# Signalsmith-Audio/signalsmith-stretch

Measured on AMD Instinct MI355X. Metric: Msamples/sec (in+out) at 48kHz stereo presetDefault, higher is better.
Workload: dtype f32

## Files before the change

### signalsmith-stretch_amd/csrc/smst_fft.hip

```cpp
#include "smst_kernels_common.h"
#include <type_traits>

namespace smst {

template <int SIGN> __device__ __forceinline__ fc mulTwiddle(fc v, fc w) { return fmul<(SIGN > 0)>(v, w); }
template <int SIGN> __device__ __forceinline__ fc addJ(fc a, fc b) { return (SIGN < 0) ? fsubI(a, b) : faddI(a, b); }
template <int SIGN> __device__ __forceinline__ fc subJ(fc a, fc b) { return (SIGN < 0) ? faddI(a, b) : fsubI(a, b); }
template <int SIGN> __device__ __forceinline__ fc mulJ(fc a) { return (SIGN < 0) ? fmake(a.y, -a.x) : fmake(-a.y, a.x); }

template <int SIGN>
__device__ __forceinline__ void dft4(fc &a, fc &b, fc &c, fc &d) {
	const fc apc = fadd(a, c), amc = fsub(a, c), bpd = fadd(b, d), bmd = fsub(b, d);
	a = fadd(apc, bpd);
	b = addJ<SIGN>(amc, bmd);
	c = fsub(apc, bpd);
	d = subJ<SIGN>(amc, bmd);
}
template <int SIGN>
__device__ __forceinline__ void dft4J(fc &a, fc &b, fc &c, fc &d) {
	const fc apc = addJ<SIGN>(a, c), amc = subJ<SIGN>(a, c), bpd = fadd(b, d), bmd = fsub(b, d);
	a = fadd(apc, bpd);
	b = addJ<SIGN>(amc, bmd);
	c = fsub(apc, bpd);
	d = subJ<SIGN>(amc, bmd);
}
template <int SIGN>
__device__ __forceinline__ void dft3(fc &a, fc &b, fc &c) {
	const float s3 = 0.86602540378443864676f;
	const fc bpc = fadd(b, c), bmc = fsub(b, c);
	const fc t = fmake(a.x - 0.5f*bpc.x, a.y - 0.5f*bpc.y);
	const fc jb = mulJ<SIGN>(bmc);
	const fc u = fmake(jb.x*s3, jb.y*s3);
	a = fadd(a, bpc);
	b = fadd(t, u);
	c = fsub(t, u);
}
template <int SIGN>
__device__ __forceinline__ void dft5(fc &a, fc &b, fc &c, fc &d, fc &e) {
	const float c1 = 0.30901699437494742410f, c2 = -0.80901699437494742410f;
	const float s1 = 0.95105651629515357212f, s2 = 0.58778525229247312917f;
	const fc bpe = fadd(b, e), bme = fsub(b, e), cpd = fadd(c, d), cmd = fsub(c, d);
	const fc t1 = fmake(a.x + c1*bpe.x + c2*cpd.x, a.y + c1*bpe.y + c2*cpd.y);
	const fc t2 = fmake(a.x + c2*bpe.x + c1*cpd.x, a.y + c2*bpe.y + c1*cpd.y);
	const fc u1 = fmake(s1*bme.x + s2*cmd.x, s1*bme.y + s2*cmd.y);
	const fc u2 = fmake(s2*bme.x - s1*cmd.x, s2*bme.y - s1*cmd.y);
	a = fadd(a, fadd(bpe, cpd));
	b = addJ<SIGN>(t1, u1);
	c = addJ<SIGN>(t2, u2);
	d = subJ<SIGN>(t2, u2);
	e = subJ<SIGN>(t1, u1);
}
template <int SIGN>
__device__ float2 *fftLds(float2 *src2, float2 *dst2, const FftPlan &plan, const float2 *__restrict__ tw2) {
	fc *src = reinterpret_cast<fc *>(src2), *dst = reinterpret_cast<fc *>(dst2);
	const fc *__restrict__ tw = reinterpret_cast<const fc *>(tw2);
	const int H = plan.H;
	int nCur = H;
	int shift = 0;
	for (int pass = 0; pass < plan.npass; ++pass) {
		const int r = plan.radix[pass];
		const int m = nCur/r;
		const int nb = H/r;
		const int twScale = H/nCur;
		if (r == 4) {
			const int s = 1 << shift;
			for (int t = threadIdx.x; t < nb; t += blockDim.x) {
				const int p = t >> shift, q0 = t & (s - 1);
				const fc *in = src + q0 + (p << shift);
				const int inStride = m << shift;
				fc *out = dst + q0 + ((4*p) << shift);
				fc a = in[0], b = in[inStride], c = in[2*inStride], e = in[3*inStride];
				dft4<SIGN>(a, b, c, e);
				const int ti = p*twScale;
				out[0] = a;
				out[s] = mulTwiddle<SIGN>(b, tw[ti]);
				out[2*s] = mulTwiddle<SIGN>(c, tw[2*ti]);
				out[3*s] = mulTwiddle<SIGN>(e, tw[3*ti]);
			}
			shift += 2;
		} else if (r == 2) {
			const int s = 1 << shift;
			for (int t = threadIdx.x; t < nb; t += blockDim.x) {
				const int p = t >> shift, q0 = t & (s - 1);
				const fc *in = src + q0 + (p << shift);
				const int inStride = m << shift;
				fc *out = dst + q0 + ((2*p) << shift);
				const fc a = in[0], b = in[inStride];
				out[0] = fadd(a, b);
				out[s] = mulTwiddle<SIGN>(fsub(a, b), tw[p*twScale]);
			}
			shift += 1;
		} else if (r == 3) {
			const int s = nb;
			for (int t = threadIdx.x; t < nb; t += blockDim.x) {
				fc a = src[t], b = src[t + s], c = src[t + 2*s];
				dft3<SIGN>(a, b, c);
				dst[t] = a;
				dst[t + s] = b;
				dst[t + 2*s] = c;
			}
		} else {
			const int s = nb;
			for (int t = threadIdx.x; t < nb; t += blockDim.x) {
				fc a = src[t], b = src[t + s], c = src[t + 2*s], e = src[t + 3*s], f = src[t + 4*s];
				dft5<SIGN>(a, b, c, e, f);
				dst[t] = a;
				dst[t + s] = b;
				dst[t + 2*s] = c;
				dst[t + 3*s] = e;
				dst[t + 4*s] = f;
			}
		}
		__syncthreads();
		fc *tmp = src; src = dst; dst = tmp;
		nCur = m;
	}
	return reinterpret_cast<float2 *>(src);
}

template <int SIGN>
__device__ __forceinline__ fc mulConst(fc v, float re, float im) {
	const float s = (SIGN < 0) ? -im : im;
	return fmake(v.x*re - v.y*s, v.x*s + v.y*re);
}
template <int SIGN>
__device__ __forceinline__ void dft16(fc (&v)[16]) {
#pragma unroll
	for (int i = 0; i < 4; ++i) dft4<SIGN>(v[i], v[i + 4], v[i + 8], v[i + 12]);
	const float c1 = 0.92387953251128675613f, s1 = 0.38268343236508977173f, h = 0.70710678118654752440f;
	v[1 + 4] = mulConst<SIGN>(v[1 + 4], c1, s1);
	v[1 + 8] = mulConst<SIGN>(v[1 + 8], h, h);
	v[1 + 12] = mulConst<SIGN>(v[1 + 12], s1, c1);
	v[2 + 4] = mulConst<SIGN>(v[2 + 4], h, h);
	v[2 + 12] = mulConst<SIGN>(v[2 + 12], -h, h);
	v[3 + 4] = mulConst<SIGN>(v[3 + 4], s1, c1);
	v[3 + 8] = mulConst<SIGN>(v[3 + 8], -h, h);
	v[3 + 12] = mulConst<SIGN>(v[3 + 12], -c1, -s1);
#pragma unroll
	for (int e = 0; e < 4; ++e) {
		if (e == 2) dft4J<SIGN>(v[4*e], v[4*e + 1], v[4*e + 2], v[4*e + 3]);
		else dft4<SIGN>(v[4*e], v[4*e + 1], v[4*e + 2], v[4*e + 3]);
	}
}
template <int SIGN, int RA, int N>
__device__ __forceinline__ void dftPow2(fc (&v)[N], int base, int stride) {
	if constexpr (RA == 2) {
		const fc a = v[base], b = v[base + stride];
		v[base] = fadd(a, b);
		v[base + stride] = fsub(a, b);
	} else if constexpr (RA == 4) {
		dft4<SIGN>(v[base], v[base + stride], v[base + 2*stride], v[base + 3*stride]);
	} else {
		static_assert(RA == 8, "radix 2, 4 or 8");
		fc e0 = v[base], e1 = v[base + 2*stride], e2 = v[base + 4*stride], e3 = v[base + 6*stride];
		fc o0 = v[base + stride], o1 = v[base + 3*stride], o2 = v[base + 5*stride], o3 = v[base + 7*stride];
		dft4<SIGN>(e0, e1, e2, e3);
		dft4<SIGN>(o0, o1, o2, o3);
		const float h = 0.70710678118654752440f;
		o1 = mulConst<SIGN>(o1, h, h);
		o3 = mulConst<SIGN>(o3, -h, h);
		v[base] = fadd(e0, o0); v[base + 4*stride] = fsub(e0, o0);
		v[base + stride] = fadd(e1, o1); v[base + 5*stride] = fsub(e1, o1);
		v[base + 2*stride] = addJ<SIGN>(e2, o2); v[base + 6*stride] = subJ<SIGN>(e2, o2);
		v[base + 3*stride] = fadd(e3, o3); v[base + 7*stride] = fsub(e3, o3);
	}
}
template <int R3> struct LastStage {
	static constexpr int G = (R3%3 == 0) ? 3 : 5;
	static constexpr int RA = R3/G;
	static_assert(R3%G == 0 && (RA == 2 || RA == 4 || RA == 8), "last stage: {2,4,8} x {3,5} points");
};
template <int SIGN, int R3>
__device__ __forceinline__ void dftLast(fc (&v)[R3]) {
	constexpr int G = LastStage<R3>::G, RA = LastStage<R3>::RA;
#pragma unroll
	for (int i = 0; i < G; ++i) dftPow2<SIGN, RA>(v, i, G);
#pragma unroll
	for (int i = 1; i < G; ++i) {
#pragma unroll
		for (int e = 1; e < RA; ++e) {
			const float ang = 6.28318530717958647692f*float(i*e)/float(R3);
			v[i + G*e] = mulConst<SIGN>(v[i + G*e], __builtin_cosf(ang), __builtin_sinf(ang));
		}
	}
#pragma unroll
	for (int e = 0; e < RA; ++e) {
		if constexpr (G == 3) dft3<SIGN>(v[G*e], v[G*e + 1], v[G*e + 2]);
		else dft5<SIGN>(v[G*e], v[G*e + 1], v[G*e + 2], v[G*e + 3 < R3 ? G*e + 3 : 0], v[G*e + 4 < R3 ? G*e + 4 : 0]);
	}
}

struct BlockSync { __device__ __forceinline__ void operator()() const { __syncthreads(); } };
struct NoHook { __device__ __forceinline__ void operator()() const {} };
struct NoArrival { __device__ __forceinline__ fc operator()(fc v, int) const { return v; } };
template <int FRAMES> struct FrameSet { fc f[FRAMES]; };
struct StageTwiddles { float4 w[8]; };
struct TwiddlesFromTable {};
template <int SIGN, int R3, bool LEAN, int ROUNDS = 0, int FRAMES = 1, typename Load, typename Prep, typename Store, typename Sync = BlockSync, typename LastRead = NoHook,
          typename Requested = NoHook, typename FirstWritten = NoHook, typename Arrived = NoArrival, typename TwRegs = TwiddlesFromTable>
__device__ __forceinline__ void fftFast(float2 *lds2, const float4 *__restrict__ twA, const float4 *__restrict__ twB, Load load, Prep prep, Store store,
                                        const int t = threadIdx.x, Sync sync = Sync(), LastRead lastRead = LastRead(), Requested requested = Requested(),
                                        FirstWritten firstWritten = FirstWritten(), Arrived arrived = Arrived(), TwRegs twRegs = TwRegs()) {
	static_assert(FRAMES == 1 || FRAMES == 2, "one frame, or two in lockstep");
	constexpr int MA = 16*R3, BUF = 17*MA;
	constexpr bool TW_REGS = std::is_same<TwRegs, StageTwiddles>::value;
	static_assert(!(TW_REGS && LEAN), "the lean tables have no register form");
	fc *lds = reinterpret_cast<fc *>(lds2);
	auto prepOf = [&](int j, int idx, int f) { if constexpr (FRAMES == 1) return prep(j, idx); else return prep(j, idx, f); };
	auto storeOf = [&](int j, fc u, auto r, int idx, int f) { if constexpr (FRAMES == 1) store(j, u, r, idx); else store(j, u, r, idx, f); };
	fc v[FRAMES][16];
	if (t < MA) {
#pragma unroll
		for (int k = 0; k < 16; ++k) {
			if constexpr (FRAMES == 1) v[0][k] = load(t + MA*k, k);
			else {
				const FrameSet<FRAMES> both = load(t + MA*k, k);
#pragma unroll
				for (int f = 0; f < FRAMES; ++f) v[f][k] = both.f[f];
			}
		}
	}
	requested();
	if (t < MA) {
#pragma unroll
		for (int f = 0; f < FRAMES; ++f) {
#pragma unroll
			for (int k = 0; k < 16; ++k) {
				if constexpr (FRAMES == 1) v[f][k] = arrived(v[f][k], t + MA*k);
				else v[f][k] = arrived(v[f][k], t + MA*k, k, f);
			}
		}
		fc w[16];
		if constexpr (LEAN) {
			const float4 a = twA[t], b = twA[MA + t], c = twA[2*MA + t];
			w[1] = fmake(a.x, a.y); w[2] = fmake(a.z, a.w); w[3] = fmake(b.x, b.y); w[4] = fmake(b.z, b.w);
			w[8] = fmake(c.x, c.y); w[12] = fmake(c.z, c.w);
#pragma unroll
			for (int hi = 4; hi <= 12; hi += 4) {
#pragma unroll
				for (int lo = 1; lo < 4; ++lo) w[hi + lo] = fmul<false>(w[hi], w[lo]);
			}
		} else {
			float4 wA[8];
#pragma unroll
			for (int i = 0; i < 8; ++i) {
				if constexpr (TW_REGS) wA[i] = twRegs.w[i];
				else wA[i] = twA[i*MA + t];
			}
#pragma unroll
			for (int n = 1; n < 16; ++n) {
				const float4 pr = wA[(n - 1) >> 1];
				w[n] = ((n - 1) & 1) ? fmake(pr.z, pr.w) : fmake(pr.x, pr.y);
			}
		}
#pragma unroll
		for (int f = 0; f < FRAMES; ++f) dft16<SIGN>(v[f]);
#pragma unroll
		for (int f = 0; f < FRAMES; ++f) {
#pragma unroll
			for (int pos = 0; pos < 16; ++pos) {
				const int n = (pos >> 2) + 4*(pos & 3);
				lds[f*BUF + 17*t + n] = n > 0 ? mulTwiddle<SIGN>(v[f][pos], w[n]) : v[f][pos];
			}
		}
	}
	firstWritten();
	sync();
	const int p = t >> 4, q0 = t & 15;
	if (t < MA) {
#pragma unroll
		for (int f = 0; f < FRAMES; ++f) {
#pragma unroll
			for (int k = 0; k < 16; ++k) v[f][k] = lds[f*BUF + q0 + 17*(p + R3*k)];
		}
	}
	sync();
	if (t < MA) {
		float4 wB[8];
#pragma unroll
		for (int i = 0; i < 8; ++i) wB[i] = twB[i*R3 + p];
#pragma unroll
		for (int f = 0; f < FRAMES; ++f) dft16<SIGN>(v[f]);
#pragma unroll
		for (int f = 0; f < FRAMES; ++f) {
#pragma unroll
			for (int pos = 0; pos < 16; ++pos) {
				const int n = (pos >> 2) + 4*(pos & 3);
				fc val = v[f][pos];
				if (n > 0) {
					const float4 pr = wB[(n - 1) >> 1];
					val = mulTwiddle<SIGN>(val, ((n - 1) & 1) ? fmake(pr.z, pr.w) : fmake(pr.x, pr.y));
				}
				lds[f*BUF + q0 + 256*p + 16*n] = val;
			}
		}
	}
	sync();
	if (t < 256) {
		constexpr int G = LastStage<R3>::G, RA = LastStage<R3>::RA;
		fc u[FRAMES][R3];
#pragma unroll
		for (int f = 0; f < FRAMES; ++f) {
#pragma unroll
			for (int k = 0; k < R3; ++k) u[f][k] = lds[f*BUF + t + 256*k];
		}
		lastRead();
		constexpr int CHUNK = ROUNDS ? R3/ROUNDS : (R3 <= 12 ? R3 : (R3 == 24 ? 6 : 5));
		decltype(prepOf(0, 0, 0)) ready[FRAMES][CHUNK];
#pragma unroll
		for (int f = 0; f < FRAMES; ++f) {
#pragma unroll
			for (int i = 0; i < CHUNK; ++i) {
				const int e = i/G, c = i - G*e;
				ready[f][i] = prepOf(t + 256*(e + RA*c), e + RA*c, f);
			}
		}
#pragma unroll
		for (int f = 0; f < FRAMES; ++f) dftLast<SIGN, R3>(u[f]);
#pragma unroll
		for (int f = 0; f < FRAMES; ++f) {
#pragma unroll
			for (int p0 = 0; p0 < R3; p0 += CHUNK) {
				if (p0 > 0) {
#pragma unroll
					for (int i = 0; i < CHUNK; ++i) {
						const int pos = p0 + i, e = pos/G, c = pos - G*e;
						if (pos < R3) ready[f][i] = prepOf(t + 256*(e + RA*c), e + RA*c, f);
					}
				}
#pragma unroll
				for (int i = 0; i < CHUNK; ++i) {
					const int pos = p0 + i, e = pos/G, c = pos - G*e;
					if (pos < R3) storeOf(t + 256*(e + RA*c), u[f][pos], ready[f][i], e + RA*c, f);
				}
			}
		}
	}
}

constexpr int fastBlockThreads(int R3) { return 16*R3 > 256 ? 16*R3 : 256; }

__device__ __forceinline__ bool hopWantsAnalysis(const HopDesc &hd, int which) {
	return (hd.flags & HOP_ACTIVE) && (hd.flags & HOP_NEW_SPECTRUM) && !(hd.flags & HOP_PREANALYSED) && (!which || (hd.flags & HOP_REANALYSE_PREV));
}

__device__ __forceinline__ int halfBinIndex(int j, int H, int N) {
	const int kk = 2*j;
	return kk >= H ? N - 1 - kk : kk;
}
__device__ __forceinline__ fc loadHalfBin(const float2 *X, int j, int H, int N) {
	return fconjLoad(X + halfBinIndex(j, H, N), 2*j >= H);
}
__device__ __forceinline__ void storeHalfBin(float2 *dst, int j, fc u, int H, int N) {
	fconjStore(dst + halfBinIndex(j, H, N), u, 2*j >= H);
}

__device__ __forceinline__ float2 analysisElement(float4 w, float xr, float xi, int slot) {
	float2 r = make_float2(0.f, 0.f);
	if (slot < 15) r = make_float2(xr*w.x, xr*w.y);
	if (slot > 0) r = make_float2(fmaf(xi, w.z, r.x), fmaf(xi, w.w, r.y));
	return r;
}
__device__ __forceinline__ float2 analysisSamples(const float *x0, const float *x1, int m, int slot) {
	return make_float2(slot < 15 ? x0[m] : 0.f, slot > 0 ? x1[m] : 0.f);
}
__device__ __forceinline__ float2 analysisElement(float4 w, const float *x0, const float *x1, int m, int slot) {
	const float2 x = analysisSamples(x0, x1, m, slot);
	return analysisElement(w, x.x, x.y, slot);
}
__device__ __forceinline__ fc leanModulation(float2 hb, int k, int per) {
	const float ang = 3.14159265358979323846f*float(k)/float(per);
	return fmulExpr(fpack(hb), fmake(__builtin_cosf(ang), -__builtin_sinf(ang)));
}
__device__ __forceinline__ void storeWindowed(float *dst, int m, fc u, fc tw, float wRe, float wIm, int B, int H) {
	const int halfB = B/2;
	const fc v = fmulc(u, tw);
	if (m < B - halfB) dst[m + halfB] = (2*v.x)*wRe;
	if (m >= H - halfB) dst[m - H + halfB] = (2*v.y)*wIm;
}
__device__ __forceinline__ void storeWindowed(float *dst, int m, fc u, float4 r, int B, int H) {
	storeWindowed(dst, m, u, fmake(r.x, r.y), r.z, r.w, B, H);
}

template <int R3, bool LEAN>
__global__ __launch_bounds__(fastBlockThreads(R3)) __attribute__((amdgpu_waves_per_eu(4, 4))) void kAnalyseFast(DevBatch d, IoArgs io, int sBase, int hopBase, int lateOnly) {
	extern __shared__ __attribute__((aligned(16))) unsigned char smemRaw[];
	float2 *lds = reinterpret_cast<float2 *>(smemRaw);
	const BlockCoord bc = xcdAwareBlock();
	const int k = bc.x;
	const int c = bc.y >> 1;
	const int which = bc.y & 1;
	const int s = bc.s;
	const HopDesc hd = d.hops[(size_t)(sBase + s)*d.hopStride + hopBase + k];
	if (!hopWantsAnalysis(hd, which)) return;
	if (lateOnly && analysisWindowInCall(d.B, d.M, d.I, hd.inputOffset, which, io.inSamples[sBase + s])) return;
	const int B = d.B, H = d.M, halfB = B/2, N = d.N;
	const int base = hd.inputOffset - (which ? d.I : 0) - B;
	const float *x = io.in + (size_t)(sBase + s)*io.inStreamStride + (size_t)c*io.inChannelStride;
	const float *hist = d.hist + ((size_t)(sBase + s)*d.C + c)*(size_t)d.histPitch + d.histBase[d.histCur][sBase + s] + d.histLen;
	const float2 *__restrict__ winA = d.winA, *__restrict__ winB = d.winB;
	float2 *dst = (which ? d.Xprev : d.Xcur) + rowOf(d, s, k, c);
	auto prep = [](int, int) { return 0; };
	auto store = [&](int j, fc u, int, int) { storeHalfBin(dst, j, u, H, N); };
	constexpr int MA = 16*R3;
	const float4 *__restrict__ twA = LEAN ? d.twA6 : d.twA4;
	const float2 *__restrict__ win2 = d.win2;
	const float2 hb = LEAN ? d.halfTw[min((int)threadIdx.x, MA - 1)] : make_float2(0.f, 0.f);
	if (base >= 0 && H - halfB == MA && B - halfB == 15*MA) {
		const float *x0 = x + base + halfB, *x1 = x + base - H + halfB;
		const float4 *__restrict__ win4 = d.win4;
		fftFast<-1, R3, LEAN>(lds, twA, d.twB4,
			[&](int m, int slot) {
				if constexpr (LEAN) {
					const float2 w = win2[m];
					float2 z = make_float2(0.f, 0.f);
					if (slot < 15) z.x = x0[m]*w.x;
					if (slot > 0) z.y = x1[m]*w.y;
					return fmul<false>(fpack(z), leanModulation(hb, slot, 32));
				} else {
					return fpack(analysisElement(win4[m], x0, x1, m, slot));
				}
// ... 150 lines not shown
		}
		if (!on[0] && !on[1]) continue;
		auto prep = [](int, int, int = 0) { return 0; };
		if (on[0] && on[1]) {
			float4 win[16];
			[[maybe_unused]] fc landed[TWIST ? R3 : 1];
			fftFast<-1, R3, false, 0, 2>(wg.lds, nullptr, wg.twB,
				[&](int m, int slot) {
					FrameSet<2> r;
#pragma unroll
					for (int f = 0; f < 2; ++f) r.f[f] = fpack(analysisSamples(x0[f], x1[f], m, slot));
					return r;
				},
				prep, [&](int j, fc u, int, int idx, int f) {
					if constexpr (TWIST) {
						const fc landedValue = fconjIf(u, 2*j >= H);
						float2 *row = dst[f] + halfBinIndex(j, H, N);
						if (f == 0) { landed[idx] = landedValue; *reinterpret_cast<fc *>(row) = landedValue; }
						else *row = prevHopTwist(funpack(landed[idx]), funpack(landedValue), rotOf[idx]);
					} else {
						storeHalfBin(dst[f], j, u, H, N);
					}
				}, t, sync, NoHook(),
				[&]() {
#pragma unroll
					for (int slot = 0; slot < 16; ++slot) win[slot] = wg.table[tA + MA*slot];
					asm volatile("" ::: "memory");
				},
				NoHook(), [&](fc x, int, int slot, int) { return fpack(analysisElement(win[slot], x.x, x.y, slot)); }, twA);
		} else {
			const int f = on[0] ? 0 : 1;
			const float *xa = x0[f], *xb = x1[f];
			float2 *dstOne = dst[f];
			fftFast<-1, R3, false>(wg.lds, nullptr, wg.twB,
				[&](int m, int slot) { return fpack(analysisElement(wg.table[tA + MA*slot], xa, xb, m, slot)); },
				prep, [&](int j, fc u, int, int) { storeHalfBin(dstOne, j, u, H, N); }, t, sync, NoHook(), NoHook(), NoHook(), NoArrival(), twA);
		}
		sync();
	}
}

__global__ __launch_bounds__(256) void kTwistRows(DevBatch d, IoArgs io, int sBase, int hopBase, int teams) {
	const int k = blockIdx.x, c = blockIdx.y, s = blockIdx.z;
	const HopDesc hd = d.hops[(size_t)(sBase + s)*d.hopStride + hopBase + k];
	if (!hopWantsAnalysis(hd, 1)) return;
	const int nIn = io.inSamples[sBase + s];
	if (teams && analysisWindowInCall(d.B, d.M, d.I, hd.inputOffset, 0, nIn) && analysisWindowInCall(d.B, d.M, d.I, hd.inputOffset, 1, nIn)) return;
	const float2 *cur = d.Xcur + rowOf(d, s, k, c);
	float2 *prev = d.Xprev + rowOf(d, s, k, c);
	for (int b = threadIdx.x; b < d.M; b += blockDim.x) prev[b] = prevHopTwist(cur[b], prev[b], d.rot[b]);
}

template <int R3, bool LEAN>
__global__ __launch_bounds__(fastBlockThreads(R3)) void kSynthFast(DevBatch d, int sBase, int hopBase) {
	extern __shared__ __attribute__((aligned(16))) unsigned char smemRaw[];
	float2 *lds = reinterpret_cast<float2 *>(smemRaw);
	const int k = blockIdx.x, c = blockIdx.y, s = blockIdx.z;
	const HopDesc hd = d.hops[(size_t)(sBase + s)*d.hopStride + hopBase + k];
	if (!(hd.flags & HOP_ACTIVE)) return;
	const int B = d.B, H = d.M, N = d.N;
	const float2 *X = d.OUT + rowOf(d, s, k, c);
	float *__restrict__ frame = frameOf(d, s, k, c);
	auto loadBin = [&](int j, int) { return loadHalfBin(X, j, H, N); };
	if constexpr (LEAN) {
		const float2 *__restrict__ win2 = d.win2;
		const float2 hb = d.halfTw[min((int)threadIdx.x, 255)];
		fftFast<+1, R3, true>(lds, d.twA6, d.twB4, loadBin,
			[&](int m, int) { return win2[m]; },
			[&](int m, fc u, float2 w, int j) { storeWindowed(frame, m, u, leanModulation(hb, j, 2*R3), w.x, w.y, B, H); });
	} else {
		const float4 *__restrict__ synTab = d.synTab;
		fftFast<+1, R3, false>(lds, d.twA4, d.twB4, loadBin,
			[&](int m, int) {
				return synTab[m];
			},
			[&](int m, fc u, float4 r, int) { storeWindowed(frame, m, u, r, B, H); });
	}
}

template <int R3, int TEAMS>
__global__ __launch_bounds__(256*TEAMS) void kSynthTeams(DevBatch d, const HopDesc *__restrict__ hopTable, int sBase, int hopBase, int tileHops, int nStreams) {
	extern __shared__ __attribute__((aligned(16))) unsigned char smemRaw[];
	constexpr int H = 256*R3, N = 2*H;
	const int B = d.B;
	const int total = tileHops*d.C*nStreams;
	TeamWorkgroup<R3, TEAMS> wg(smemRaw, d, d.synTab);
	const TeamSync sync = wg.sync();
	const int stride = gridDim.x*TEAMS;
	for (int lin = blockIdx.x + gridDim.x*wg.team; lin < total; lin += stride) {
		const BlockCoord bc = xcdAwareCoord(lin, tileHops, d.C, nStreams);
		const HopDesc hd = hopTable[(size_t)(sBase + bc.s)*d.hopStride + hopBase + bc.x];
		if (!(hd.flags & HOP_ACTIVE)) continue;
		const float2 *X = d.OUT + rowOf(d, bc.s, bc.x, bc.y);
		float *__restrict__ frame = frameOf(d, bc.s, bc.x, bc.y);
		fftFast<+1, R3, false>(wg.lds, wg.twA, wg.twB,
			[&](int j, int) { return loadHalfBin(X, j, H, N); },
			[&](int m, int) { return wg.table[m]; },
			[&](int m, fc u, float4 r, int) { storeWindowed(frame, m, u, r, B, H); }, wg.t, sync);
		sync();
	}
}

__device__ __forceinline__ float carriedSumAt(const DevBatch &d, size_t row, int i) { return i < d.carryLen ? loadCarrySum(d, d.carryCur, row + i) : 0.0f; }
__device__ __forceinline__ float carriedProductAt(const DevBatch &d, const float *__restrict__ carryWpOld, int i) { return i < d.carryLen ? carryWpOld[i] : 1e-30f; }
struct FrameRange { int lo, hi; };
__device__ __forceinline__ FrameRange coveringFrames(int relFirst, int relLast, int B, int I, int hopCount) {
	FrameRange r;
	r.hi = (relLast >= 0) ? relLast/I : -1;
	r.lo = (relFirst - B + 1 > 0) ? (relFirst - B + 1 + I - 1)/I : 0;
	if (r.hi > hopCount - 1) r.hi = hopCount - 1;
	return r;
}
__device__ __forceinline__ float windowProductAt(const DevBatch &d, const EmitDesc &ed, const float *__restrict__ carryWpOld, int i) {
	float wp = carriedProductAt(d, carryWpOld, i);
	if (ed.hopCount > 0) {
		const int rel = ed.nLo + i - ed.firstHopPos - d.delta;
		const FrameRange q = coveringFrames(rel, rel, d.B, d.I, ed.hopCount);
		for (int k = q.lo; k <= q.hi; ++k) wp += d.wprod[rel - k*d.I];
	}
	return wp;
}
__global__ __launch_bounds__(256) void kEmitProducts(DevBatch d, int sBase, int tileIndex) {
	const int sg = sBase + blockIdx.y;
	const EmitDesc ed = d.emit[(size_t)sg*d.emitStride + tileIndex];
	const int span = ed.nHi - ed.nLo, CL = d.carryLen;
	const float *carryWpOld = d.carryWp[d.carryCur] + carryWpRow(d, sg) + d.carryBase[d.carryCur][sg];
	const int i = blockIdx.x*blockDim.x + threadIdx.x;
	if (i == 0) d.carryBase[d.carryCur ^ 1][sg] = 0;
	if (i < d.wpHeadLen) d.wpHead[(size_t)sg*d.wpHeadLen + i] = windowProductAt(d, ed, carryWpOld, i);
	else if (i - d.wpHeadLen < CL) d.carryWp[d.carryCur ^ 1][carryWpRow(d, sg) + (i - d.wpHeadLen)] = windowProductAt(d, ed, carryWpOld, span + (i - d.wpHeadLen));
}

struct SynthEmitEdge {
	EmitDesc ed;
	float *out;
	size_t carryRow;
	size_t carried;
	const float *wpOld;
};
__device__ __forceinline__ SynthEmitEdge synthEmitEdge(const DevBatch &d, const IoArgs &io, int sg, int c, int tileIndex) {
	SynthEmitEdge e;
	e.ed = d.emit[(size_t)sg*d.emitStride + tileIndex];
	const int carryFrom = d.carryBase[d.carryCur][sg];
	e.carryRow = carrySumRow(d, sg, c);
	e.carried = e.carryRow + carryFrom;
	e.wpOld = d.carryWp[d.carryCur] + carryWpRow(d, sg) + carryFrom;
	e.out = io.out + (size_t)sg*io.outStreamStride + (size_t)c*io.outChannelStride;
	return e;
}
__device__ __forceinline__ void synthEmitPlace(const DevBatch &d, const SynthEmitEdge &e, int n, float sum, float wp) {
	if (n < e.ed.nHi) e.out[n] = sum/wp;
	else if (n - e.ed.nHi < d.carryLen) storeCarrySum(d, d.carryCur ^ 1, e.carryRow + (n - e.ed.nHi), sum);
}
template <int R3, int QN, int SLOTS, bool SPLIT, int GI, int GB>
__global__ __launch_bounds__(512) void kSynthEmitTeams(DevBatch d, IoArgs io, int sBase, int tileIndex, int nStreams) {
	constexpr int TEAMS = 2, MA = 16*R3, H = 256*R3, N = 2*H, NI = QN + 1, DQ = SPLIT ? 1 : 0;
	static_assert(GI == 0 || (GI <= 256*SLOTS && GI > 256*(SLOTS - 1) && QN*GI >= GB && GB <= N), "the geometry this instantiation is for");
	extern __shared__ __attribute__((aligned(16))) unsigned char smemRaw[];
	const int B = GI ? GB : d.B, I = GI ? GI : d.I;
	TeamWorkgroup<R3, TEAMS> wg(smemRaw, d, d.synTab);
	const TeamSync sync = wg.sync();
	const int team = wg.team, t = wg.t;
	float2 *lds = wg.lds;
	float *ex = reinterpret_cast<float *>(lds);
	auto inInterval = [&](int slot) { return 256*slot + t < I; };
	auto inFrame = [&](int a, int slot) { return 256*slot + t < I && a*I + 256*slot + t < B; };
	float steady[SLOTS];
#pragma unroll
	for (int slot = 0; slot < SLOTS; ++slot) {
		steady[slot] = 1e-30f;
#pragma unroll
		for (int a = QN - 1; a >= 0; --a) {
			if (inFrame(a, slot)) steady[slot] += d.wprod[a*I + 256*slot + t];
		}
		keepUnconditional(steady[slot]);
	}
	const int C = d.C, items = nStreams*C;
	const unsigned hopPitch = (unsigned)C*(unsigned)d.Mp;
	for (int item = blockIdx.x*TEAMS + team; item < items; item += gridDim.x*TEAMS) {
		const int s = item/C, c = item - s*C, sg = sBase + s;
		int cnt, off, firstHopPos;
		float acc[NI][SLOTS];
		{
			const SynthEmitEdge e = synthEmitEdge(d, io, sg, c, tileIndex);
			const int CL = d.carryLen;
			cnt = e.ed.hopCount;
			if (cnt == 0) {
				const int span = e.ed.nHi - e.ed.nLo;
				for (int i = t; i < span + CL; i += 256) synthEmitPlace(d, e, e.ed.nLo + i, carriedSumAt(d, e.carried, i), carriedProductAt(d, e.wpOld, i));
				continue;
			}
			firstHopPos = e.ed.firstHopPos;
			off = firstHopPos - e.ed.nLo;
			for (int i = t; i < off; i += 256) synthEmitPlace(d, e, e.ed.nLo + i, carriedSumAt(d, e.carried, i), carriedProductAt(d, e.wpOld, i));
#pragma unroll
			for (int u = 0; u < NI; ++u) {
#pragma unroll
				for (int slot = 0; slot < SLOTS; ++slot) {
					const int i = off + u*I + 256*slot + t;
					acc[u][slot] = inInterval(slot) ? carriedSumAt(d, e.carried, i) : 0.0f;
				}
			}
		}
#pragma unroll
		for (int u = 0; u < NI; ++u) {
#pragma unroll
			for (int slot = 0; slot < SLOTS; ++slot) keepUnconditional(acc[u][slot]);
		}
		const float2 *spectra = d.OUT + rowOf(d, s, 0, c);
		float *outHops = io.out + (size_t)sg*io.outStreamStride + (size_t)c*io.outChannelStride + firstHopPos;
		const float *wpHead = d.wpHead + (size_t)sg*d.wpHeadLen + off;
		auto overlapAdd = [&]() {
			float e[QN][SLOTS];
			int tt = t;
			keepUnconditional(tt);
#pragma unroll
			for (int a = 0; a < QN; ++a) {
#pragma unroll
				for (int slot = 0; slot < SLOTS; ++slot) {
					if (GI && (256*slot >= GI || a*GI + 256*slot >= GB)) continue;
					e[a][slot] = ex[inFrame(a, slot) ? a*I + 256*slot + tt : 0];
				}
			}
#pragma unroll
			for (int a = 0; a < QN; ++a) {
#pragma unroll
				for (int slot = 0; slot < SLOTS; ++slot) {
					if (GI && (256*slot >= GI || a*GI + 256*slot >= GB)) continue;
					keepUnconditional(e[a][slot]);
					acc[a + DQ][slot] = inFrame(a, slot) ? acc[a + DQ][slot] + e[a][slot] : acc[a + DQ][slot];
				}
			}
		};
		auto moveRing = [&]() {
#pragma unroll
			for (int u = 0; u + 1 < NI; ++u) {
#pragma unroll
				for (int slot = 0; slot < SLOTS; ++slot) acc[u][slot] = acc[u + 1][slot];
			}
#pragma unroll
			for (int slot = 0; slot < SLOTS; ++slot) acc[NI - 1][slot] = 0.0f;
		};
		auto productsOf = [&](int q, float (&wp)[SLOTS]) {
#pragma unroll
			for (int slot = 0; slot < SLOTS; ++slot) wp[slot] = steady[slot];
			if (q < NI) {
				Async4 head[SLOTS];
				const float *from = wpHead + q*I;
#pragma unroll
				for (int slot = 0; slot < SLOTS; ++slot) asyncLoad4(head[slot], from + (inInterval(slot) ? 256*slot + t : 0));
				asyncWait<0>();
#pragma unroll
				for (int slot = 0; slot < SLOTS; ++slot) {
					asyncArrived(head[slot]);
					if (inInterval(slot)) wp[slot] = asyncValue(head[slot]);
				}
			}
		};
		auto emitFinal = [&](int q) {
			float wp[SLOTS];
			productsOf(q, wp);
			float *to = outHops + q*I;
#pragma unroll
			for (int slot = 0; slot < SLOTS; ++slot) {
				if (inInterval(slot)) to[256*slot + t] = acc[0][slot]/wp[slot];
			}
			moveRing();
		};
		Async8 next[16];
#pragma unroll
		for (int k = 0; k < 16; ++k) asyncClear(next[k]);
		auto request = [&](int q) {
			const float2 *X = spectra + (unsigned)q*hopPitch;
			if (t < MA) {
#pragma unroll
				for (int k = 0; k < 16; ++k) asyncLoad8(next[k], X + halfBinIndex(t + MA*k, H, N));
			}
		};
		auto landed = [&]() {
			asyncWait<0>();
#pragma unroll
			for (int k = 0; k < 16; ++k) asyncArrived(next[k]);
		};
		request(0);
		landed();
		for (int q = 0; q < cnt; ++q) {
			fftFast<+1, R3, false, 2>(lds, wg.twA, wg.twB,
				[&](int, int k) { return fpack(asyncValue(next[k])); },
				[&](int m, int) { return wg.table[m]; },
				[&](int m, fc u, float4 r, int) { storeWindowed(ex, m, u, r, B, H); }, t, sync, sync,
				[&]() {
					if (q > 0) overlapAdd();
					sync();
				},
				[&]() {
					if (q > 0) emitFinal(q - 1);
					request(q + 1 < cnt ? q + 1 : q);
				},
				[&](fc v, int j) { return fconjIf(v, 2*j >= H); });
			sync();
			landed();
		}
		overlapAdd();
		sync();
		int sgE = sg, cE = c;
		keepUnconditional(sgE);
		keepUnconditional(cE);
		const SynthEmitEdge e = synthEmitEdge(d, io, __builtin_amdgcn_readfirstlane(sgE), __builtin_amdgcn_readfirstlane(cE), tileIndex);
		auto emitEdge = [&](int q) {
			float wp[SLOTS];
			productsOf(q, wp);
			const int n0 = firstHopPos + q*I;
#pragma unroll
			for (int slot = 0; slot < SLOTS; ++slot) {
				if (inInterval(slot)) synthEmitPlace(d, e, n0 + 256*slot + t, acc[0][slot], wp[slot]);
			}
			moveRing();
		};
		emitEdge(cnt - 1);
		const bool trailing = SPLIT && firstHopPos + cnt*I < e.ed.nHi;
		if (trailing) emitEdge(cnt);
		const int n0 = firstHopPos + (cnt + (trailing ? 1 : 0))*I;
#pragma unroll
		for (int u = 0; u < NI; ++u) {
#pragma unroll
			for (int slot = 0; slot < SLOTS; ++slot) {
				if (inInterval(slot)) synthEmitPlace(d, e, n0 + u*I + 256*slot + t, acc[u][slot], 1.0f);
			}
		}
	}
}

__global__ __launch_bounds__(256) void kEnergy(DevBatch d, IoArgs io, int sBase, float *__restrict__ energyOut) {
	const int s = blockIdx.x, part = blockIdx.y, parts = gridDim.y;
	if (part == 0 && (int)threadIdx.x >= parts && (int)threadIdx.x < kEnergyParts) energyOut[(size_t)(sBase + s)*kEnergyParts + threadIdx.x] = 0.0f;
	const int n = io.inSamples[sBase + s];
	const int lo = (int)((long long)n*part/parts), hi = (int)((long long)n*(part + 1)/parts);
	float acc = 0;
	for (int c = 0; c < d.C; ++c) {
		const float *x = io.in + (size_t)(sBase + s)*io.inStreamStride + (size_t)c*io.inChannelStride;
		for (int i = lo + threadIdx.x; i < hi; i += blockDim.x) {
			float v = x[i];
			acc += v*v;
		}
	}
	extern __shared__ __attribute__((aligned(16))) unsigned char smemRaw[];
	float *red = reinterpret_cast<float *>(smemRaw);
	red[threadIdx.x] = acc;
	__syncthreads();
	for (int w = 128; w > 0; w >>= 1) {
		if ((int)threadIdx.x < w) red[threadIdx.x] += red[threadIdx.x + w];
		__syncthreads();
	}
	if (threadIdx.x == 0) energyOut[(size_t)(sBase + s)*kEnergyParts + part] = red[0];
}

template <bool BIG>
__global__ __launch_bounds__(256) void kAnalyse(DevBatch d, IoArgs io, int sBase, int hopBase) {
	extern __shared__ __attribute__((aligned(16))) unsigned char smemRaw[];
	float2 *bufA = reinterpret_cast<float2 *>(smemRaw);
	float2 *bufB = bufA + d.M;

	const BlockCoord bc = xcdAwareBlock();
	const int k = bc.x;
	const int c = bc.y >> 1;
	const int which = bc.y & 1;
	const int s = bc.s;
	const HopDesc hd = d.hops[(size_t)(sBase + s)*d.hopStride + hopBase + k];
	if (!hopWantsAnalysis(hd, which)) return;

	const int B = d.B, H = d.M, halfB = B/2;
	const int base = hd.inputOffset - (which ? d.I : 0) - B;
	const float *x = io.in + (size_t)(sBase + s)*io.inStreamStride + (size_t)c*io.inChannelStride;
	const float *hist = d.hist + ((size_t)(sBase + s)*d.C + c)*(size_t)d.histPitch + d.histBase[d.histCur][sBase + s];
	const float *__restrict__ win = d.window;
	float2 *dst = (which ? d.Xprev : d.Xcur) + rowOf(d, s, k, c);
	if (BIG) bufB = dst;

	for (int m = threadIdx.x; m < H; m += blockDim.x) {
		float re = 0, im = 0;
		if (m < B - halfB) {
			int i = m + halfB;
			int src = base + i;
			float v = (src >= 0) ? x[src] : hist[d.histLen + src];
			re = v*win[i];
		}
		if (m >= H - halfB) {
			int i = m - H + halfB;
			int src = base + i;
			float v = (src >= 0) ? x[src] : hist[d.histLen + src];
			im = v*win[i];
		}
		bufA[m] = funpack(fmul<false>(fmake(re, im), fpack(d.halfTw[m])));
	}
	__syncthreads();
	float2 *res = fftLds<-1>(bufA, bufB, d.plan, d.twH);
	if (BIG && res == dst) {
		for (int j = threadIdx.x; j < H; j += blockDim.x) bufA[j] = dst[j];
		__syncthreads();
		res = bufA;
	}
	const int N = d.N;
	for (int j = threadIdx.x; j < H; j += blockDim.x) storeHalfBin(dst, j, fpack(res[j]), H, N);
}

template <bool BIG>
__global__ __launch_bounds__(256) void kSynth(DevBatch d, int sBase, int hopBase) {
	extern __shared__ __attribute__((aligned(16))) unsigned char smemRaw[];
	float2 *bufA = reinterpret_cast<float2 *>(smemRaw);
	float2 *bufB = bufA + d.M;
	const int k = blockIdx.x, c = blockIdx.y, s = blockIdx.z;
	if (BIG) bufB = d.fftScratch + rowOf(d, s, k, c);
	const HopDesc hd = d.hops[(size_t)(sBase + s)*d.hopStride + hopBase + k];
	if (!(hd.flags & HOP_ACTIVE)) return;
	const int B = d.B, H = d.M, N = d.N, halfB = B/2;
	const float2 *X = d.OUT + rowOf(d, s, k, c);
	for (int j = threadIdx.x; j < H; j += blockDim.x) bufA[j] = funpack(loadHalfBin(X, j, H, N));
	__syncthreads();
	float2 *res = fftLds<+1>(bufA, bufB, d.plan, d.twH);
	float *frame = frameOf(d, s, k, c);
	const float *__restrict__ win = d.window;
	for (int m = threadIdx.x; m < H; m += blockDim.x) {
		const float wRe = (m < B - halfB) ? win[m + halfB] : 0.0f, wIm = (m >= H - halfB) ? win[m - H + halfB] : 0.0f;
		storeWindowed(frame, m, fpack(res[m]), fpack(d.halfTw[m]), wRe, wIm, B, H);
	}
}

template <int KMAX>
__global__ __launch_bounds__(256) void kEmit(DevBatch d, IoArgs io, int sBase, int tileIndex) {
	const int s = blockIdx.z, sg = sBase + s, c = blockIdx.y;
	const EmitDesc ed = d.emit[(size_t)sg*d.emitStride + tileIndex];
	const int span = ed.nHi - ed.nLo;
	const int i0 = 4*(blockIdx.x*blockDim.x + threadIdx.x);
	const int CL = d.carryLen;
	const int total = span + CL;
	if (i0 >= total) return;
	const int B = d.B, I = d.I;
	const int carryFrom = d.carryBase[d.carryCur][sg];
	const size_t carryRow = carrySumRow(d, sg, c);
	const float *carryWpOld = d.carryWp[d.carryCur] + carryWpRow(d, sg) + carryFrom;
	if (i0 == 0 && c == 0) d.carryBase[d.carryCur ^ 1][sg] = 0;
	float sum[4], wp[4];
	if (i0 + 3 < CL && !d.halfState) {
		const float4 a = *reinterpret_cast<const float4 *>(d.carrySum[d.carryCur] + carryRow + carryFrom + i0), b = *reinterpret_cast<const float4 *>(carryWpOld + i0);
		sum[0] = a.x; sum[1] = a.y; sum[2] = a.z; sum[3] = a.w;
		wp[0] = b.x; wp[1] = b.y; wp[2] = b.z; wp[3] = b.w;
	} else {
#pragma unroll
		for (int j = 0; j < 4; ++j) {
			const int i = i0 + j;
			sum[j] = carriedSumAt(d, carryRow + carryFrom, i);
			wp[j] = carriedProductAt(d, carryWpOld, i);
// ... 200 lines not shown
```

Measured before the change: 51570.

## Load synth spectra with scalar-base immediates and fold conjugation into first DFT4

The synthesis kernel now issues its half-spectrum loads as global_load_dwordx2 with a uniform scalar base and compile-time immediate offsets, replacing per-element halfBinIndex address computation. The conjugation of the upper half-bins is folded into the first radix-4 butterflies via packed-add neg modifiers instead of a separate conditional conjugate. Loaded values enter the FFT only at the arrival hook, and register lifetimes are cut after the first stage. This lowers VALU address arithmetic and register pressure in the load path, at the cost of inline asm that depends on a fixed index pattern and the 13-bit offset limit.

After: 51930 (median of 6 runs). About the same (+0.7%).

```diff
diff --git a/signalsmith-stretch_amd/csrc/smst_async_sbase.h b/signalsmith-stretch_amd/csrc/smst_async_sbase.h
--- /dev/null
+++ b/signalsmith-stretch_amd/csrc/smst_async_sbase.h
@@ -0,0 +1,12 @@
+#pragma once
+#include <smst_async.h>
+
+namespace smst {
+
+template <int IMM>
+__device__ __forceinline__ void asyncLoad8Scalar(Async8 &r, const void *base, unsigned laneBytes) {
+	static_assert(IMM >= -4096 && IMM <= 4095, "the instruction's immediate offset: 13 bits, signed");
+	asm volatile("global_load_dwordx2 %0, %1, %2 offset:%3" : "=&v"(r.v) : "v"(laneBytes), "s"(base), "n"(IMM) : "memory");
+}
+
+}
diff --git a/signalsmith-stretch_amd/csrc/smst_fft.hip b/signalsmith-stretch_amd/csrc/smst_fft.hip
--- a/signalsmith-stretch_amd/csrc/smst_fft.hip
+++ b/signalsmith-stretch_amd/csrc/smst_fft.hip
@@ -1,5 +1,8 @@
 #include "smst_kernels_common.h"
+#include <smst_fft_conj.h>
+#include <smst_async_sbase.h>
 #include <type_traits>
+#include <utility>
 
 namespace smst {
 
@@ -8,9 +11,10 @@
 template <int SIGN> __device__ __forceinline__ fc subJ(fc a, fc b) { return (SIGN < 0) ? faddI(a, b) : fsubI(a, b); }
 template <int SIGN> __device__ __forceinline__ fc mulJ(fc a) { return (SIGN < 0) ? fmake(a.y, -a.x) : fmake(-a.y, a.x); }
 
-template <int SIGN>
+template <int SIGN, bool CONJ_CD = false>
 __device__ __forceinline__ void dft4(fc &a, fc &b, fc &c, fc &d) {
-	const fc apc = fadd(a, c), amc = fsub(a, c), bpd = fadd(b, d), bmd = fsub(b, d);
+	const fc apc = CONJ_CD ? faddConj(a, c) : fadd(a, c), amc = CONJ_CD ? fsubConj(a, c) : fsub(a, c);
+	const fc bpd = CONJ_CD ? faddConj(b, d) : fadd(b, d), bmd = CONJ_CD ? fsubConj(b, d) : fsub(b, d);
 	a = fadd(apc, bpd);
 	b = addJ<SIGN>(amc, bmd);
 	c = fsub(apc, bpd);
@@ -123,10 +127,10 @@
 	const float s = (SIGN < 0) ? -im : im;
 	return fmake(v.x*re - v.y*s, v.x*s + v.y*re);
 }
-template <int SIGN>
+template <int SIGN, bool CONJ_UPPER = false>
 __device__ __forceinline__ void dft16(fc (&v)[16]) {
 #pragma unroll
-	for (int i = 0; i < 4; ++i) dft4<SIGN>(v[i], v[i + 4], v[i + 8], v[i + 12]);
+	for (int i = 0; i < 4; ++i) dft4<SIGN, CONJ_UPPER>(v[i], v[i + 4], v[i + 8], v[i + 12]);
 	const float c1 = 0.92387953251128675613f, s1 = 0.38268343236508977173f, h = 0.70710678118654752440f;
 	v[1 + 4] = mulConst<SIGN>(v[1 + 4], c1, s1);
 	v[1 + 8] = mulConst<SIGN>(v[1 + 8], h, h);
@@ -192,7 +196,8 @@
 
 struct BlockSync { __device__ __forceinline__ void operator()() const { __syncthreads(); } };
 struct NoHook { __device__ __forceinline__ void operator()() const {} };
-struct NoArrival { __device__ __forceinline__ fc operator()(fc v, int) const { return v; } };
+struct NoArrival { __device__ __forceinline__ fc operator()(fc v, int, int) const { return v; } };
+template <bool CONJ_UPPER = false> struct InArrived {};
 template <int FRAMES> struct FrameSet { fc f[FRAMES]; };
 struct StageTwiddles { float4 w[8]; };
 struct TwiddlesFromTable {};
@@ -205,6 +210,9 @@
 	constexpr int MA = 16*R3, BUF = 17*MA;
 	constexpr bool TW_REGS = std::is_same<TwRegs, StageTwiddles>::value;
 	static_assert(!(TW_REGS && LEAN), "the lean tables have no register form");
+	constexpr bool CONJ_UPPER = std::is_same<decltype(load(0, 0)), InArrived<true>>::value;
+	constexpr bool IN_ARRIVED = CONJ_UPPER || std::is_same<decltype(load(0, 0)), InArrived<false>>::value;
+	static_assert(!IN_ARRIVED || FRAMES == 1, "elements that enter in `arrived`: the one-frame form");
 	fc *lds = reinterpret_cast<fc *>(lds2);
 	auto prepOf = [&](int j, int idx, int f) { if constexpr (FRAMES == 1) return prep(j, idx); else return prep(j, idx, f); };
 	auto storeOf = [&](int j, fc u, auto r, int idx, int f) { if constexpr (FRAMES == 1) store(j, u, r, idx); else store(j, u, r, idx, f); };
@@ -212,8 +220,9 @@
 	if (t < MA) {
 #pragma unroll
 		for (int k = 0; k < 16; ++k) {
-			if constexpr (FRAMES == 1) v[0][k] = load(t + MA*k, k);
-			else {
+			if constexpr (FRAMES == 1) {
+				if constexpr (!IN_ARRIVED) v[0][k] = load(t + MA*k, k);
+			} else {
 				const FrameSet<FRAMES> both = load(t + MA*k, k);
 #pragma unroll
 				for (int f = 0; f < FRAMES; ++f) v[f][k] = both.f[f];
@@ -226,7 +235,8 @@
 		for (int f = 0; f < FRAMES; ++f) {
 #pragma unroll
 			for (int k = 0; k < 16; ++k) {
-				if constexpr (FRAMES == 1) v[f][k] = arrived(v[f][k], t + MA*k);
+				if constexpr (IN_ARRIVED) v[f][k] = arrived(fmake(0.f, 0.f), t + MA*k, k);
+				else if constexpr (FRAMES == 1) v[f][k] = arrived(v[f][k], t + MA*k, k);
 				else v[f][k] = arrived(v[f][k], t + MA*k, k, f);
 			}
 		}
@@ -254,7 +264,7 @@
 			}
 		}
 #pragma unroll
-		for (int f = 0; f < FRAMES; ++f) dft16<SIGN>(v[f]);
+		for (int f = 0; f < FRAMES; ++f) dft16<SIGN, CONJ_UPPER>(v[f]);
 #pragma unroll
 		for (int f = 0; f < FRAMES; ++f) {
 #pragma unroll
@@ -267,6 +277,10 @@
 	firstWritten();
 	sync();
 	const int p = t >> 4, q0 = t & 15;
+	if constexpr (IN_ARRIVED) {
+#pragma unroll
+		for (int k = 0; k < 16; ++k) fcNoValue(v[0][k]);
+	}
 	if (t < MA) {
 #pragma unroll
 		for (int f = 0; f < FRAMES; ++f) {
@@ -723,6 +737,12 @@
 	if (n < e.ed.nHi) e.out[n] = sum/wp;
 	else if (n - e.ed.nHi < d.carryLen) storeCarrySum(d, d.carryCur ^ 1, e.carryRow + (n - e.ed.nHi), sum);
 }
+template <int MA, int... K>
+__device__ __forceinline__ void requestHalfBinRow(Async8 (&next)[16], const char *row, unsigned lowerBytes, unsigned upperBytes, std::integer_sequence<int, K...>) {
+	static_assert(16*MA <= 4095, "a step of k within the immediate offset");
+	((K < 8 ? asyncLoad8Scalar<16*MA*(K%3 - 1)>(next[K], row + 48*MA*(K/3), lowerBytes)
+	        : asyncLoad8Scalar<16*MA*((15 - K)%3 - 1)>(next[K], row + 48*MA*((15 - K)/3), upperBytes)), ...);
+}
 template <int R3, int QN, int SLOTS, bool SPLIT, int GI, int GB>
 __global__ __launch_bounds__(512) void kSynthEmitTeams(DevBatch d, IoArgs io, int sBase, int tileIndex, int nStreams) {
 	constexpr int TEAMS = 2, MA = 16*R3, H = 256*R3, N = 2*H, NI = QN + 1, DQ = SPLIT ? 1 : 0;
@@ -778,7 +798,7 @@
 #pragma unroll
 			for (int slot = 0; slot < SLOTS; ++slot) keepUnconditional(acc[u][slot]);
 		}
-		const float2 *spectra = d.OUT + rowOf(d, s, 0, c);
+		const float2 *spectra = d.OUT + rowOf(d, __builtin_amdgcn_readfirstlane(s), 0, __builtin_amdgcn_readfirstlane(c));
 		float *outHops = io.out + (size_t)sg*io.outStreamStride + (size_t)c*io.outChannelStride + firstHopPos;
 		const float *wpHead = d.wpHead + (size_t)sg*d.wpHeadLen + off;
 		auto overlapAdd = [&]() {
@@ -841,12 +861,10 @@
 		Async8 next[16];
 #pragma unroll
 		for (int k = 0; k < 16; ++k) asyncClear(next[k]);
+		const unsigned lowerBytes = 16*MA + 16*t, upperBytes = 32*MA - 8 - 16*t;
 		auto request = [&](int q) {
-			const float2 *X = spectra + (unsigned)q*hopPitch;
-			if (t < MA) {
-#pragma unroll
-				for (int k = 0; k < 16; ++k) asyncLoad8(next[k], X + halfBinIndex(t + MA*k, H, N));
-			}
+			const char *row = reinterpret_cast<const char *>(spectra + (unsigned)q*hopPitch);
+			if (t < MA) requestHalfBinRow<MA>(next, row, lowerBytes, upperBytes, std::make_integer_sequence<int, 16>());
 		};
 		auto landed = [&]() {
 			asyncWait<0>();
@@ -857,7 +875,7 @@
 		landed();
 		for (int q = 0; q < cnt; ++q) {
 			fftFast<+1, R3, false, 2>(lds, wg.twA, wg.twB,
-				[&](int, int k) { return fpack(asyncValue(next[k])); },
+				[](int, int) { return InArrived<true>(); },
 				[&](int m, int) { return wg.table[m]; },
 				[&](int m, fc u, float4 r, int) { storeWindowed(ex, m, u, r, B, H); }, t, sync, sync,
 				[&]() {
@@ -868,7 +886,7 @@
 					if (q > 0) emitFinal(q - 1);
 					request(q + 1 < cnt ? q + 1 : q);
 				},
-				[&](fc v, int j) { return fconjIf(v, 2*j >= H); });
+				[&](fc, int, int k) { return fpack(asyncValue(next[k])); });
 			sync();
 			landed();
 		}
diff --git a/signalsmith-stretch_amd/csrc/smst_fft_conj.h b/signalsmith-stretch_amd/csrc/smst_fft_conj.h
--- /dev/null
+++ b/signalsmith-stretch_amd/csrc/smst_fft_conj.h
@@ -0,0 +1,18 @@
+#pragma once
+#include <smst_fft_complex.h>
+
+namespace smst {
+
+__device__ __forceinline__ fc faddConj(fc a, fc b) {
+	fc r;
+	asm("v_pk_add_f32 %0, %1, %2 neg_hi:[0,1]" : "=v"(r) : "v"(a), "v"(b));
+	return r;
+}
+__device__ __forceinline__ fc fsubConj(fc a, fc b) {
+	fc r;
+	asm("v_pk_add_f32 %0, %1, %2 neg_lo:[0,1]" : "=v"(r) : "v"(a), "v"(b));
+	return r;
+}
+__device__ __forceinline__ void fcNoValue(fc &a) { asm volatile("" : "=v"(a)); }
+
+}
```
